# MGI-tech-bioinformatics/SuperPlus

Hardware: AMD Instinct MI355X
Metric: k-mers/s (DF createDict stage: trim + canonical k-mer count + solid filter + spectrum + adjacency) (higher is better)
Workload: dtype u64

## Files before the change

superplus_amd/csrc/dfk.hip:

```cpp
#include "../../include/dfk.h"
#include "dfk_kernels.h"

#include <algorithm>
#include <chrono>
#include <cstdarg>
#include <cstdio>
#include <cstdlib>
#include <cstring>
#include <atomic>
#include <fcntl.h>
#include <functional>
#include <new>
#include <string>
#include <sys/mman.h>
#include <sys/stat.h>
#include <unistd.h>
#include <condition_variable>
#include <memory>
#include <mutex>
#include <thread>
#include <vector>

using namespace dfk;

namespace {

thread_local std::string g_err;

int fail(int code, const char* fmt, ...)
{
    char buf[512];
    va_list ap; va_start(ap, fmt); vsnprintf(buf, sizeof buf, fmt, ap); va_end(ap);
    g_err = buf;
    return code;
}

#define HIP_TRY(expr) do { hipError_t e_ = (expr); if (e_ != hipSuccess) \
    return fail(DFK_E_HIP, "%s failed: %s (%s:%d)", #expr, hipGetErrorString(e_), __FILE__, __LINE__); } while (0)

template <class F> int guarded(F&& f)
{
    try { return f(); }
    catch (const std::bad_alloc&) { return fail(DFK_E_NOMEM, "out of host memory"); }
    catch (const std::exception& e) { return fail(DFK_E_HIP, "internal error: %s", e.what()); }
    catch (...) { return fail(DFK_E_HIP, "internal error"); }
}

struct DevBuf {
    void* p = nullptr; size_t bytes = 0;
    bool sub = false;
};

bool g_trace = getenv("DFK_TRACE") != nullptr;
#define TRACE(...) do { if (g_trace) { fprintf(stderr, "[dfk] " __VA_ARGS__); fputc('\n', stderr); fflush(stderr); } } while (0)
inline double wall_now() { return std::chrono::duration<double>(std::chrono::steady_clock::now().time_since_epoch()).count(); }

template <int K> struct CountCfg;
#ifndef DFK_LOG2S
#define DFK_LOG2S 11
#endif
#ifndef DFK_NWAVES
#define DFK_NWAVES 8
#endif
template <> struct CountCfg<40> { static constexpr int LOG2S = DFK_LOG2S, NWAVES = DFK_NWAVES; };
template <> struct CountCfg<48> { static constexpr int LOG2S = DFK_LOG2S, NWAVES = DFK_NWAVES; };
template <> struct CountCfg<60> { static constexpr int LOG2S = DFK_LOG2S, NWAVES = DFK_NWAVES; };

struct Inputs {
    const uint8_t* packed; uint64_t packed_bytes;
    const uint64_t* base_off; const uint32_t* read_len;
    const uint8_t* pq; uint64_t pq_bytes; const uint64_t* pq_off;
    const int32_t* bc; uint64_t n_reads;
};

}

struct dfk_ctx {
    dfk_config cfg{};
    int device = 0;
    hipStream_t stream = nullptr;
    hipStream_t stream2 = nullptr;
    hipDeviceProp_t prop{};
    uint64_t budget = 0, held = 0, peak = 0;
    struct Owned { void* p; uint64_t bytes, seq; };
    std::vector<Owned> owned;
    uint64_t alloc_seq = 0;
    bool have = false;
    uint64_t n_reads = 0;
    struct FileRange { const char* base; uint64_t bytes; int fd; uint64_t off; };
    std::vector<FileRange> file_ranges;
    DevBuf good_len;
    struct Part { DevBuf buf, pre; uint64_t n = 0; uint64_t blist = 0, n_blist = 0; bool listed = false; };
    bool want_blist = false;
    int pending_blist = -1;
    std::function<int()> after_count_launch;
    std::vector<Part> parts;
    uint64_t n_solid = 0, n_boundary = 0;
    unsigned seg_attempt = 0;
    double distinct_per_inst = 0.0;
    double plan_derate = 0.95;
    std::vector<int64_t> hist;
    std::vector<dfk_entry32> sorted, sorted_pre;
    bool sorted_ok = false, sorted_pre_ok = false;
    dfk_stats st{};
    bool shard_open = false, shard_use_bc = false;
    const void* sh_in[7] = {};
    uint64_t sh_packed_bytes = 0, sh_pq_bytes = 0, sh_n_reads = 0, sh_n_inst_local = 0;
    int64_t sh_read_id0 = 0;
    DevBuf shard_send[2];
    uint32_t shard_send_pass[2] = {~0u, ~0u};
    DevBuf shard_recv[2];
    unsigned shard_recv_seq = 0;
    uint64_t budget_taken = 0;
    void* sh_staged[6] = {};
    uint64_t sh_b0 = 0, sh_b1 = 0, sh_q0 = 0, sh_q1 = 0, sh_staged_reads = 0;
    DevBuf adj_keys, adj_src; uint64_t adj_n = 0;
    DevBuf set; uint64_t set_mask = 0;
    double t_upload_done = 0;
    uint32_t shard_world = 1, shard_log2_nb = 0;
    void* shard_state = nullptr;
    void (*shard_state_free)(void*) = nullptr;
    void* lane_pool = nullptr; void (*lane_pool_free)(void*) = nullptr;
    std::mutex lane_mu;
    void* graph_state = nullptr;
    void (*graph_state_free)(void*) = nullptr;
    unsigned int* d_resident = nullptr;
    unsigned int resident_target = 0;
    unsigned int last_wg_idle = 0;
    void* kept[6] = {};
    uint64_t kept_packed_bytes = 0, kept_pq_bytes = 0, kept_n_reads = 0, kept_budget = 0;

    struct Free { uint64_t off, bytes; };
    struct Chunk { char* p; uint64_t bytes; std::vector<Free> free_list; bool adopted = false; };
    std::vector<Chunk> chunks;
    uint64_t reserved = 0;

    uint64_t first_chunk_hint = 0;
    bool carve(Chunk& k, size_t bytes, DevBuf& b, bool long_lived)
    {
        if (!long_lived) {
            for (size_t i = k.free_list.size(); i-- > 0;)
                if (k.free_list[i].bytes >= bytes) {
                    k.free_list[i].bytes -= bytes;
                    b.p = k.p + k.free_list[i].off + k.free_list[i].bytes; b.bytes = bytes;
                    if (!k.free_list[i].bytes) k.free_list.erase(k.free_list.begin() + i);
                    return true;
                }
            return false;
        }
// ... 579 lines not shown
    }
    unsigned int bad = 0;
    HIP_TRY(hipMemcpy(&bad, J->d_bad.p, 4, hipMemcpyDeviceToHost));
    c->release(J->d_bad); c->release(J->cur);
    if (bad) return fail(DFK_E_HIP, "scatter: %u buckets did not receive the records counted for them (run summaries and bucket counters disagree)", bad);
    TRACE("scatter of buckets [%u, %u) done (%llu records, %llu items)", J->lo, J->lo + J->n,
          (unsigned long long)J->P.n_records, (unsigned long long)J->P.n_items);
    return 0;
}

constexpr int E_SPLIT_NO_ROOM = -101;
constexpr int E_SEGMENT_FULL = -100;

struct CountRun {
    CountGlobals* g = nullptr; uint4* seg = nullptr; unsigned long long* hist = nullptr;
    CountParams cp{}; unsigned grid = 0;
    DevBuf big; uint64_t big_cap = 0;
    DevBuf d_hist, d_g;
    DevBuf d_snap;
    DevBuf d_part;
    DevBuf d_wg;
    uint64_t solid_seen = 0, inst_seen = 0;
    uint64_t boundary_seen = 0;
    uint64_t splits_seen = 0;
};

int count_run_begin(dfk_ctx* c, CountRun* R)
{
    int rc = c->alloc(R->d_hist, (uint64_t)HIST_GLOBAL_BINS * 8, "spectrum bins", true); if (rc) return rc;
    rc = c->alloc(R->d_g, sizeof(CountGlobals), "count globals", true); if (rc) return rc;
    HIP_TRY(hipMemsetAsync(R->d_hist.p, 0, (uint64_t)HIST_GLOBAL_BINS * 8, c->stream));
    HIP_TRY(hipMemsetAsync(R->d_g.p, 0, sizeof(CountGlobals), c->stream));
    R->g = (CountGlobals*)R->d_g.p; R->hist = (unsigned long long*)R->d_hist.p;
    return c->alloc(R->d_snap, (uint64_t)HIST_GLOBAL_BINS * 8 + 256, "spectrum snapshot", true);
}

int count_snapshot(dfk_ctx* c, CountRun* R, bool restore)
{
    char* snap = (char*)R->d_snap.p;
    const uint64_t hb = (uint64_t)HIST_GLOBAL_BINS * 8;
    if (!restore) {
        HIP_TRY(hipMemcpyAsync(snap, R->d_hist.p, hb, hipMemcpyDeviceToDevice, c->stream));
        HIP_TRY(hipMemcpyAsync(snap + hb, R->d_g.p, sizeof(CountGlobals), hipMemcpyDeviceToDevice, c->stream));
    } else {
        HIP_TRY(hipMemcpyAsync(R->d_hist.p, snap, hb, hipMemcpyDeviceToDevice, c->stream));
        HIP_TRY(hipMemcpyAsync(R->d_g.p, snap + hb, sizeof(CountGlobals), hipMemcpyDeviceToDevice, c->stream));
    }
    return 0;
}

int count_run_end(dfk_ctx* c, CountRun* R)
{
    CountGlobals hg{};
    HIP_TRY(hipMemcpy(&hg, R->d_g.p, sizeof hg, hipMemcpyDeviceToHost));
    c->st.n_distinct = hg.n_distinct; c->n_boundary = hg.n_boundary;
#ifdef DFK_PHASE_TIMES
    {
        unsigned long long ph[16] = {};
        (void)hipMemcpyFromSymbol(ph, HIP_SYMBOL(g_phase), sizeof ph);
        unsigned long long tot = 0; for (int i = 0; i < 12; ++i) tot += ph[i];
        static const char* nm[12] = {"item loop tail (thread 0 publishes)", "barrier: item start", "chunks (stage + insert)", "barrier: chunks done", "finish pass 1 (solidity)", "barrier", "finish pass 2 (adjacency look-ups)", "barrier", "finish pass 3 (emit)", "barrier", "clear + reduce", "drain"};
        fprintf(stderr, "[dfk] k_count wave cycles by phase (%.3e memtime ticks in all):\n", (double)tot);
        for (int i = 0; i < 12; ++i) fprintf(stderr, "[dfk]   %5.1f %%  %s\n", 100.0 * (double)ph[i] / (double)std::max(1ull, tot), nm[i]);
        unsigned long long z[16] = {};
        (void)hipMemcpyToSymbol(HIP_SYMBOL(g_phase), z, sizeof z);
    }
#endif
    DevBuf d_max; int rc = c->alloc(d_max, 16, "max bin"); if (rc) return rc;
    HIP_TRY(hipMemsetAsync(d_max.p, 0, 16, c->stream));
    hipLaunchKernelGGL(k_hist_max, dim3(1024), dim3(256), 0, c->stream, (const unsigned long long*)R->d_hist.p, HIST_GLOBAL_BINS,
                       (unsigned int*)d_max.p);
    uint32_t nb = 0;
    HIP_TRY(hipMemcpyAsync(&nb, d_max.p, 4, hipMemcpyDeviceToHost, c->stream));
    HIP_TRY(hipStreamSynchronize(c->stream));
    c->hist.assign(nb, 0);
    if (nb) HIP_TRY(hipMemcpy(c->hist.data(), R->d_hist.p, 8ull * nb, hipMemcpyDeviceToHost));
    TRACE("spectrum read back: %u bins, %llu solid", nb, (unsigned long long)c->n_solid);
    c->release(d_max); c->release(R->d_hist); c->release(R->d_g); c->release(R->d_snap);
    return 0;
}

template <int K> unsigned count_grid(const dfk_ctx* c, int nbc = 1)
{
    constexpr int LOG2S = CountCfg<K>::LOG2S, NW = CountCfg<K>::NWAVES;
    const size_t lds = count_lds_bytes<K, LOG2S, NW, 1>() + (size_t)(nbc > 1 ? nbc - 1 : 0) * sizeof(uint32_t) * (1u << LOG2S);
    const unsigned per_cu = (unsigned)std::max<size_t>(1, (size_t)(160 * 1024) / lds);
    return (unsigned)c->prop.multiProcessorCount * per_cu;
}

int launch_boundary_list(dfk_ctx* c)
{
    if (c->pending_blist < 0) return 0;
    const dfk_ctx::Part& part = c->parts[(size_t)c->pending_blist];
    c->pending_blist = -1;
    unsigned long long* ctl = (unsigned long long*)((char*)part.buf.p + part.blist);
    HIP_TRY(hipMemsetAsync(ctl, 0, 16, c->stream2));
    hipLaunchKernelGGL(k_boundary_list, dim3((unsigned)std::min<uint64_t>((part.n + 2047) / 2048, 4096)), dim3(256), 0, c->stream2,
                       (const uint4*)part.buf.p, part.n, (uint32_t*)(ctl + 2), part.n_blist, ctl);
    HIP_TRY(hipGetLastError());
    return 0;
}

template <int K, int NBC>
int launch_count(dfk_ctx* c, const Partition& P, const ItemRange* d_items, uint64_t n_items, const CountRun& R,
                 std::vector<ItemRange>* overflowed, float* kernel_ms, const uint32_t* d_sub = nullptr, bool single_kmer_records = false)
{
    constexpr int LOG2S = CountCfg<K>::LOG2S, NW = CountCfg<K>::NWAVES;
    if (n_items == 0) return 0;
    if (n_items >= (1ull << 32)) return fail(DFK_E_ARG, "too many work items in one pass");
    DevBuf d_ovf;
    int rc = c->alloc(d_ovf, n_items * sizeof(ItemRange), "overflow list"); if (rc) return rc;
    HIP_TRY(hipMemsetAsync(&R.g->next_item, 0, 8, c->stream));
    HIP_TRY(hipMemsetAsync(&R.g->n_wg_idle, 0, 4, c->stream));
    CountParams cp = R.cp; cp.n_items = (uint32_t)n_items; cp.single = single_kmer_records ? 1u : 0u;
    const size_t lds = count_lds_bytes<K, LOG2S, NW, NBC>();
    auto kern = d_sub ? k_count<K, LOG2S, NW, NBC, true> : k_count<K, LOG2S, NW, NBC, false>;
    HIP_TRY(hipFuncSetAttribute(reinterpret_cast<const void*>(kern), hipFuncAttributeMaxDynamicSharedMemorySize, (int)lds));
    TRACE("k_count: %llu items, grid %u, lds %zu, seg_cap %llu", (unsigned long long)n_items, R.grid, lds, (unsigned long long)R.cp.seg_cap);
    Timer tk(c->stream);
    tk.start();
    hipLaunchKernelGGL(kern, dim3(R.grid), dim3(NW * 64), lds, c->stream,
                       (const uint4*)P.records.p, d_items, (const uint64_t*)P.base.p, cp, R.g, R.seg, (WgOut*)R.d_wg.p, R.hist,
                       (ItemRange*)d_ovf.p, d_sub, c->d_resident);
    HIP_TRY(hipGetLastError());
    c->resident_target += R.grid;
    if (c->after_count_launch || c->pending_blist >= 0) {
        hipLaunchKernelGGL(k_gate, dim3(1), dim3(64), 0, c->stream2, (const unsigned int*)c->d_resident, c->resident_target, 200000ull, c->d_resident + 1);
    }
    if (c->after_count_launch) { std::function<int()> f; f.swap(c->after_count_launch); rc = f(); if (rc) return rc; }
    rc = launch_boundary_list(c); if (rc) return rc;
    *kernel_ms += tk.stop();
    CountGlobals g{};
    HIP_TRY(hipMemcpyAsync(&g, R.g, sizeof g, hipMemcpyDeviceToHost, c->stream));
    HIP_TRY(hipStreamSynchronize(c->stream));
    c->last_wg_idle = g.n_wg_idle;
    if (g.n_overflow) {
        const size_t at = overflowed->size();
        overflowed->resize(at + g.n_overflow);
        HIP_TRY(hipMemcpy(overflowed->data() + at, d_ovf.p, sizeof(ItemRange) * g.n_overflow, hipMemcpyDeviceToHost));
    }
    c->release(d_ovf);
    return 0;
}

template <int K, int NBC>
int launch_count_big(dfk_ctx* c, const Partition& P, const std::vector<ItemRange>& singles, CountRun& R)
{
    constexpr int KW = KTraits<K>::KW, NW = 8;
    const uint32_t n = (uint32_t)singles.size();
    std::vector<uint32_t> idx(2 * n);
    for (uint32_t i = 0; i < n; ++i) { idx[2 * i] = singles[i].b0; idx[2 * i + 1] = singles[i].b1; }
    DevBuf d_idx, d_val;
    int rc = c->alloc(d_idx, 8ull * n, "gather index"); if (rc) return rc;
    rc = c->alloc(d_val, 16ull * n, "gather values"); if (rc) return rc;
    HIP_TRY(hipMemcpyAsync(d_idx.p, idx.data(), 8ull * n, hipMemcpyHostToDevice, c->stream));
    hipLaunchKernelGGL(k_gather_u64, dim3((2 * n + 255) / 256), dim3(256), 0, c->stream, (const uint64_t*)P.ipre.p,
                       (const uint32_t*)d_idx.p, 2 * n, (uint64_t*)d_val.p);
    HIP_TRY(hipGetLastError());
    std::vector<uint64_t> val(2 * n);
    HIP_TRY(hipMemcpyAsync(val.data(), d_val.p, 16ull * n, hipMemcpyDeviceToHost, c->stream));
    HIP_TRY(hipStreamSynchronize(c->stream));
    c->release(d_idx); c->release(d_val);
    std::vector<BigItem> items; uint64_t words = 0, tot_inst = 0;
    std::vector<uint64_t> chunk_pre(n + 1, 0), slot_pre(n + 1, 0), rec(2 * n);
    {
        DevBuf d_i2, d_v2;
        rc = c->alloc(d_i2, 8ull * n, "gather index"); if (rc) return rc;
        rc = c->alloc(d_v2, 16ull * n, "gather values"); if (rc) return rc;
        HIP_TRY(hipMemcpyAsync(d_i2.p, idx.data(), 8ull * n, hipMemcpyHostToDevice, c->stream));
        hipLaunchKernelGGL(k_gather_u64, dim3((2 * n + 255) / 256), dim3(256), 0, c->stream, (const uint64_t*)P.base.p,
                           (const uint32_t*)d_i2.p, 2 * n, (uint64_t*)d_v2.p);
        HIP_TRY(hipGetLastError());
        HIP_TRY(hipMemcpyAsync(rec.data(), d_v2.p, 16ull * n, hipMemcpyDeviceToHost, c->stream));
        HIP_TRY(hipStreamSynchronize(c->stream));
        c->release(d_i2); c->release(d_v2);
    }
    for (uint32_t i = 0; i < n; ++i) {
        tot_inst += val[2 * i + 1] - val[2 * i];
        chunk_pre[i + 1] = chunk_pre[i] + (rec[2 * i + 1] - rec[2 * i] + COUNT_CHUNK - 1) / COUNT_CHUNK;
    }
    double per_inst = c->distinct_per_inst > 0.0 ? std::min(1.0, std::max(0.05, 1.5 * c->distinct_per_inst)) : 1.0;
    DevBuf d_items, d_fail, d_pre;
    {
        const uint64_t more = tot_inst / std::max<uint32_t>(1, c->cfg.min_freq) + 1;
        if (!R.big.p) { R.big_cap = more; rc = c->alloc(R.big, R.big_cap * 32, "fallback solid entries"); if (rc) return rc; }
        else {
            CountGlobals g0{};
            HIP_TRY(hipMemcpy(&g0, R.d_g.p, sizeof g0, hipMemcpyDeviceToHost));
            DevBuf grown;
            rc = c->alloc(grown, (g0.big_cursor + more) * 32, "fallback solid entries"); if (rc) return rc;
// ... 1374 lines not shown
```

superplus_amd/csrc/dfk_kernels.h:

```cpp
#pragma once
#include <type_traits>
#include "dfk_device.h"

namespace dfk {

template <int K>
__global__ void __launch_bounds__(256)
k_trim(const uint8_t* __restrict__ pq, const uint64_t* __restrict__ pq_off, uint64_t pq_nbytes,
       const uint64_t* __restrict__ base_off, uint64_t packed_bytes, const uint32_t* __restrict__ read_len,
       uint64_t n_reads, uint32_t min_qual, uint32_t* __restrict__ good_len,
       unsigned long long* __restrict__ n_inst, unsigned int* __restrict__ bad,
       unsigned long long* __restrict__ sum_good)
{
    unsigned long long mine = 0, good = 0;
    bool any_bad = false;
    for (uint64_t r = (uint64_t)blockIdx.x * blockDim.x + threadIdx.x; r < n_reads; r += (uint64_t)gridDim.x * blockDim.x) {
        uint32_t gl = 0;
        uint64_t p = pq_off[r], end = pq_off[r + 1];
        uint32_t idx = 0, run = 0;
        const uint64_t b0 = base_off[r], b1 = base_off[r + 1];
        bool ok = p <= end && end <= pq_nbytes && b0 <= b1 && b1 <= packed_bytes && b1 - b0 >= ((uint64_t)read_len[r] + 3) / 4;
        if (!ok) end = p;
        while (p < end) {
            uint32_t nQs = pq[p];
// ... 14 lines not shown
                    const uint64_t by = bit >> 3;
                    const uint32_t sh = (uint32_t)(bit & 7);
                    uint64_t w = 0;
                    if (by + 8 <= pq_nbytes) __builtin_memcpy(&w, pq + by, 8);
                    else for (uint32_t k = 0; k < 8 && by + k < pq_nbytes; ++k) w |= (uint64_t)pq[by + k] << (8 * k);
                    w >>= sh;
                    const uint32_t n = min(left, (64u - sh) / nBits);
                    for (uint32_t i = 0; i < n; ++i, w >>= nBits) {
                        const uint32_t q = minQ + ((uint32_t)w & fmask);
                        if (q < min_qual) run = 0;
                        else if (++run >= (uint32_t)K) gl = idx + 1;
                        ++idx;
                    }
                    bit += (uint64_t)n * nBits; left -= n;
                }
            }
            p += blk;
        }
        uint32_t rl = read_len[r];
        if (!ok || idx != rl) { any_bad = true; gl = 0; }
        if (gl > rl) gl = rl;
        good_len[r] = gl;
        good += gl;
        if (gl >= (uint32_t)K + 1) mine += gl - K + 1;
    }
    __shared__ unsigned long long sh[2][4];
    __shared__ unsigned int sh_bad;
    if (threadIdx.x == 0) sh_bad = 0;
    __syncthreads();
#pragma unroll
    for (int d = 32; d > 0; d >>= 1) { mine += __shfl_down(mine, d, 64); good += __shfl_down(good, d, 64); }
    if ((threadIdx.x & 63) == 0) { sh[0][threadIdx.x >> 6] = mine; sh[1][threadIdx.x >> 6] = good; }
    if (any_bad) atomicOr(&sh_bad, 1u);
    __syncthreads();
    if (threadIdx.x == 0) {
        unsigned long long a0 = sh[0][0] + sh[0][1] + sh[0][2] + sh[0][3], a1 = sh[1][0] + sh[1][1] + sh[1][2] + sh[1][3];
        if (a0) atomicAdd(n_inst, a0);
        if (a1) atomicAdd(sum_good, a1);
        if (sh_bad) atomicOr(bad, 1u);
    }
}

struct PartParams {
    uint32_t M;
    uint32_t W;
    uint32_t log2_nb;
    uint32_t log2_world;
    int64_t  read_id0;
    uint32_t sub_lo;
    uint32_t sub_n;
    uint32_t class_mask;
};

constexpr uint32_t SWEEP_CLASSES = 32;
__host__ __device__ inline uint32_t sweep_class_of(uint32_t local_bucket, uint32_t log2_local)
{ return log2_local > 5 ? local_bucket >> (log2_local - 5) : local_bucket; }
__host__ __device__ inline uint32_t sweep_class_mask(uint32_t sub_lo, uint32_t sub_n, uint32_t log2_local)
{
    if (sub_n == 0) return 0u;
    const uint32_t a = sweep_class_of(sub_lo, log2_local), b = sweep_class_of(sub_lo + sub_n - 1, log2_local);
    const uint32_t upto_b = b >= 31 ? 0xFFFFFFFFu : ((1u << (b + 1)) - 1u);
    return upto_b & ~((1u << a) - 1u);
}

constexpr int PART_THREADS = 128;
constexpr int PART_RING = 2;
constexpr int SUMMARY_RUNS = 10;
constexpr uint32_t SUMMARY_OVERFLOW = 15;

__device__ __forceinline__ uint32_t pass_local(uint32_t bucket, const PartParams& pp)
{
    const uint32_t ls = pp.log2_nb - pp.log2_world;
    const uint32_t d = (bucket & ((1u << ls) - 1u)) - pp.sub_lo;
    return d < pp.sub_n ? (bucket >> ls) * pp.sub_n + d : 0xFFFFFFFFu;
}

__device__ __forceinline__ uint32_t bucket_of(uint32_t minhash, const PartParams& pp)
{
    const uint32_t b = (minhash * 0x9E3779B1u) >> (32 - pp.log2_nb);
    return ((b & ((1u << pp.log2_world) - 1u)) << (pp.log2_nb - pp.log2_world)) | (b >> pp.log2_world);
}
constexpr int PART_QCAP = 8;

template <int K>
__device__ __forceinline__ void emit_record(const uint32_t* __restrict__ words, uint64_t n_words, uint64_t bit0,
                                            uint32_t s0, uint32_t nk, uint32_t bucket, uint32_t gl, int32_t tag,
                                            uint64_t dst_index, uint4* __restrict__ records)
{
    const bool hp = s0 > 0;
    const bool hs = s0 + nk + (uint32_t)K <= gl;
    uint64_t bo = bit0 + 2ull * (hp ? s0 - 1 : 0);
    uint64_t wi = bo >> 5; uint32_t sh = (uint32_t)bo & 31u;
    uint32_t w[7];
#pragma unroll
    for (int i = 0; i < 7; ++i) w[i] = (wi + i < n_words) ? words[wi + i] : 0u;
    uint32_t o[6];
#pragma unroll
    for (int i = 0; i < 6; ++i) o[i] = alignbit(w[i + 1], w[i], sh);
    if (!hp) {
#pragma unroll
        for (int i = 5; i > 0; --i) o[i] = (o[i] << 2) | (o[i - 1] >> 30);
        o[0] <<= 2;
    }
    uint32_t nbits = 2u * (1u + nk + (uint32_t)K - 1u + (hs ? 1u : 0u));
#pragma unroll
    for (int i = 0; i < 6; ++i) {
        uint32_t lo = 32u * i;
        if (nbits <= lo) o[i] = 0;
        else if (nbits < lo + 32u) o[i] &= (1u << (nbits - lo)) - 1u;
    }
    uint4 a{rec_header(nk, hp, hs, bucket), (uint32_t)tag, o[0], o[1]};
    uint4 b{o[2], o[3], o[4], o[5]};
    records[2 * dst_index] = a;
    records[2 * dst_index + 1] = b;
}

constexpr uint32_t PART_CLASSES = 64;
__device__ __forceinline__ uint32_t class_bin(uint32_t bucket, const PartParams& pp)
{
    const uint32_t ls = pp.log2_nb - pp.log2_world;
    const uint32_t sub = bucket & ((1u << ls) - 1u);
    return (bucket >> ls) * PART_CLASSES + (ls > 6 ? sub >> (ls - 6) : sub);
}

template <int K, bool WRITE>
__device__ __forceinline__ void
partition_read(uint64_t r, uint32_t* smem, uint32_t* __restrict__ lh,
            const uint8_t* __restrict__ packed, uint64_t packed_bytes, const uint64_t* __restrict__ base_off,
            const uint32_t* __restrict__ good_len, const int32_t* __restrict__ bc, int64_t ign_bc_below,
            uint64_t n_reads, const PartParams& pp,
            unsigned long long* __restrict__ bucket_acc, unsigned long long* __restrict__ bucket_cur, uint64_t n_out,
            uint4* __restrict__ records, uint4* __restrict__ summaries, const uint32_t* __restrict__ read_list, uint64_t n_list,
            const uint64_t* __restrict__ slice_base, uint32_t* __restrict__ read_classes)
{
    auto place = [&](uint32_t b) -> uint64_t {
        if (!slice_base) { const uint64_t d = atomicAdd(&bucket_cur[b], 1ull); return d < n_out ? d : ~0ull; }
        const uint32_t owner = b / pp.sub_n;
        const uint64_t d = slice_base[owner] + atomicAdd(&bucket_cur[owner], 1ull);
        return d < slice_base[owner + 1] ? d : ~0ull;
    };
    uint32_t* arr = smem;
    uint32_t* queue = smem + pp.W * PART_THREADS;
    uint8_t* sidx = reinterpret_cast<uint8_t*>(smem + pp.W * PART_THREADS);
    uint32_t* ring = reinterpret_cast<uint32_t*>(sidx + pp.W * PART_THREADS);
    uint64_t sum_lo = 0, sum_hi = 0;
    const int tid = threadIdx.x;
    if (WRITE && read_list) { if (r >= n_list) return; r = read_list[r]; }
    const uint32_t M = pp.M, W = pp.W;
    const uint32_t gl = r < n_reads ? good_len[r] : 0;
    if (gl < (uint32_t)K + 1) {
        if (!WRITE && r < n_reads) { summaries[r] = uint4{0, 0, 0, 0}; if (read_classes) read_classes[r] = 0u; }
        return;
    }
    uint32_t Pi = 0, cur_rel = 0;
    uint32_t cmask = 0;
    const uint32_t log2_local = pp.log2_nb - pp.log2_world;

    const uint64_t byte0 = base_off[r];
    const uint32_t* words = reinterpret_cast<const uint32_t*>(packed);
    const uint64_t n_words = (packed_bytes + 3) >> 2;
    const uint64_t bit0 = byte0 * 8;
    int32_t tag = -1;
    if (bc && (int64_t)r + pp.read_id0 >= ign_bc_below) tag = bc[r];

    const uint32_t mmask = M == 16 ? 0xFFFFFFFFu : ((1u << (2 * M)) - 1u);
    const uint32_t rsh = 2 * (M - 1);
    uint32_t f = 0, rc = 0;
    uint32_t P = 0;
    uint32_t bi = 0;
    uint32_t cur_b = 0, cur_s0 = 0, cur_nk = 0;
    uint32_t qn = 0;

    uint64_t wi = bit0 >> 5;
    uint64_t filled_to = wi;
    auto fill = [&]() {
        uint32_t w[PART_RING];
#pragma unroll
        for (int k = 0; k < PART_RING; ++k) w[k] = filled_to + k < n_words ? words[filled_to + k] : 0u;
#pragma unroll
        for (int k = 0; k < PART_RING; ++k) ring[((filled_to + k) & (PART_RING - 1)) * PART_THREADS + tid] = w[k];
        filled_to += PART_RING;
    };
    uint32_t wbits, wnext = 0;
    if (!WRITE) { fill(); wbits = ring[(wi & (PART_RING - 1)) * PART_THREADS + tid]; }
    else { wbits = wi < n_words ? words[wi] : 0u; wnext = wi + 1 < n_words ? words[wi + 1] : 0u; }
    uint32_t wpos = (uint32_t)bit0 & 31u;
    uint32_t sfx_next = 0xFFFFFFFFu;

    auto close_run = [&]() {
        if (WRITE && cur_b == 0xFFFFFFFFu) return;
        if (!WRITE) {
            if (lh) { const uint32_t bin = class_bin(cur_b, pp); atomicAdd(&lh[bin], 1u); atomicAdd(&lh[(PART_CLASSES << pp.log2_world) + bin], cur_nk); }
            else atomicAdd(&bucket_acc[cur_b], (1ull << 32) | cur_nk);
            cmask |= 1u << sweep_class_of(cur_b & ((1u << log2_local) - 1u), log2_local);
            if (qn < (uint32_t)SUMMARY_RUNS) {
                const uint64_t fld = cur_nk | (cur_rel << 6);
                const uint32_t b = 8u + 12u * qn;
// ... 474 lines not shown
    uint32_t s0 = 0;
#pragma unroll
    for (int i = 0; i < SUMMARY_RUNS; ++i) {
        if ((uint32_t)i < n) {
            constexpr int B0 = 8;
            const int b = B0 + 12 * i;
            const uint32_t fld = (uint32_t)(b + 12 <= 64 ? lo >> b : b >= 64 ? hi >> (b - 64) : (lo >> b) | (hi << (64 - b))) & 0xFFFu;
            const uint32_t nk = fld & 63u, rel = fld >> 6;
            const uint64_t bo = bit0 + 2ull * (s0 + rel);
            const uint64_t wi = bo >> 5;
            const uint32_t w0 = words[wi], w1 = wi + 1 < n_words ? words[wi + 1] : 0u;
            const uint32_t x = alignbit(w1, w0, (uint32_t)bo & 31u) & mmask;
            uint32_t y = __brev(x);
            y = ((y >> 1) & 0x55555555u) | ((y & 0x55555555u) << 1);
            const uint32_t fw = y >> (32 - 2 * M), rcv = ~x & mmask;
            const uint32_t bucket = bucket_of(mmer_hash(fw < rcv ? fw : rcv), pp);
            const uint32_t lb = pass_local(bucket, pp);
            if (lb != 0xFFFFFFFFu) f(s0, nk, lb, bucket >> (pp.log2_nb - pp.log2_world), bit0, (uint32_t)i + 1 == n);
            s0 += nk;
        }
    }
}

template <int K>
__global__ void __launch_bounds__(256)
k_scatter_slices(const uint8_t* __restrict__ packed, uint64_t packed_bytes, const uint64_t* __restrict__ base_off,
                 const uint32_t* __restrict__ good_len, const int32_t* __restrict__ bc, int64_t ign_bc_below,
                 uint64_t n_reads, PartParams pp, const uint4* __restrict__ summaries, const uint32_t* __restrict__ read_classes,
                 const uint64_t* __restrict__ slice_base,
                 unsigned long long* __restrict__ slice_fill,
                 uint4* __restrict__ records)
{
    __shared__ uint32_t cnt[256];
    __shared__ unsigned long long at[256];
    __shared__ uint16_t list[256 * SLICE_READS];
    __shared__ uint32_t n_list;
    const uint32_t world = 1u << pp.log2_world;
    const int lane = threadIdx.x & 63;
    const uint64_t r_block = (uint64_t)blockIdx.x * 256 * SLICE_READS;
    if (threadIdx.x < world) cnt[threadIdx.x] = 0;
    if (threadIdx.x == 0) n_list = 0;
    __syncthreads();
#pragma unroll
    for (int j = 0; j < SLICE_READS; ++j) {
        const uint32_t rel = 256u * j + threadIdx.x;
        const uint64_t r = r_block + rel;
        const bool hit = r < n_reads && (!read_classes || (read_classes[r] & pp.class_mask) != 0u);
        const unsigned long long mk = __ballot(hit);
        uint32_t w = 0;
        if (lane == 0 && mk) w = atomicAdd(&n_list, (uint32_t)__popcll(mk));
        w = __builtin_amdgcn_readfirstlane(w);
        if (hit) list[w + __popcll(mk & ((1ull << lane) - 1ull))] = (uint16_t)rel;
    }
    __syncthreads();
    const uint32_t n = n_list;
    for (uint32_t i = threadIdx.x; i < n; i += 256)
        for_each_run_in_pass<K, false>(r_block + list[i], packed, packed_bytes, base_off, pp, summaries,
                                       [&](uint32_t, uint32_t, uint32_t, uint32_t owner, uint64_t, bool) { atomicAdd(&cnt[owner], 1u); });
    __syncthreads();
    if (threadIdx.x < world) {
        const uint32_t m = cnt[threadIdx.x];
        at[threadIdx.x] = slice_base[threadIdx.x] + (m ? atomicAdd(&slice_fill[threadIdx.x], (unsigned long long)m) : 0ull);
        cnt[threadIdx.x] = 0;
    }
    __syncthreads();
    const uint32_t* words = reinterpret_cast<const uint32_t*>(packed);
    const uint64_t n_words = (packed_bytes + 3) >> 2;
    (void)good_len;
    for (uint32_t i = threadIdx.x; i < n; i += 256) {
        const uint64_t r = r_block + list[i];
        int32_t tag = -1;
        if (bc && (int64_t)r + pp.read_id0 >= ign_bc_below) tag = bc[r];
        for_each_run_in_pass<K, true>(r, packed, packed_bytes, base_off, pp, summaries,
            [&](uint32_t s0, uint32_t nk, uint32_t lb, uint32_t owner, uint64_t bit0, bool last) {
                const uint64_t dst = at[owner] + atomicAdd(&cnt[owner], 1u);
                if (dst < slice_base[owner + 1]) emit_record<K>(words, n_words, bit0, s0, nk, lb, last ? 0u : 0xFFFFFFFFu, tag, dst, records);
            });
    }
}

#ifndef DFK_SWEEP_READS
#define DFK_SWEEP_READS 8
#endif
template <int K> constexpr int sweep_reads() { return KTraits<K>::KW == 4 ? 2 : DFK_SWEEP_READS; }
template <int K>
__global__ void __launch_bounds__(256)
k_scatter_runs(const uint8_t* __restrict__ packed, uint64_t packed_bytes, const uint64_t* __restrict__ base_off,
               const uint32_t* __restrict__ good_len, const int32_t* __restrict__ bc, int64_t ign_bc_below,
               uint64_t n_reads, PartParams pp, const uint4* __restrict__ summaries, const uint32_t* __restrict__ read_classes,
               unsigned long long* __restrict__ bucket_cur, uint64_t n_out, uint4* __restrict__ records)
{
    constexpr int SWEEP_READS = sweep_reads<K>();
    __shared__ uint16_t list[256 * SWEEP_READS];
    __shared__ uint32_t n_list;
    (void)good_len;
    const int lane = threadIdx.x & 63;
    const uint64_t r_block = (uint64_t)blockIdx.x * 256 * SWEEP_READS;
    if (threadIdx.x == 0) n_list = 0;
    __syncthreads();
#pragma unroll
    for (int j = 0; j < SWEEP_READS; ++j) {
        const uint32_t rel = 256u * j + threadIdx.x;
        const uint64_t r = r_block + rel;
        const bool hit = r < n_reads && (read_classes[r] & pp.class_mask) != 0u;
        const unsigned long long mk = __ballot(hit);
        uint32_t at = 0;
        if (lane == 0 && mk) at = atomicAdd(&n_list, (uint32_t)__popcll(mk));
        at = __builtin_amdgcn_readfirstlane(at);
        if (hit) list[at + __popcll(mk & ((1ull << lane) - 1ull))] = (uint16_t)rel;
    }
    __syncthreads();
    const uint32_t n = n_list;
    const uint32_t* words = reinterpret_cast<const uint32_t*>(packed);
    const uint64_t n_words = (packed_bytes + 3) >> 2;
    for (uint32_t i = threadIdx.x; i < n; i += 256) {
        const uint64_t r = r_block + list[i];
        int32_t tag = -1;
        if (bc && (int64_t)r + pp.read_id0 >= ign_bc_below) tag = bc[r];
        for_each_run_in_pass<K, true>(r, packed, packed_bytes, base_off, pp, summaries,
            [&](uint32_t s0, uint32_t nk, uint32_t lb, uint32_t, uint64_t bit0, bool last) {
                const uint64_t dst = atomicAdd(&bucket_cur[lb], 1ull);
                if (dst < n_out) emit_record<K>(words, n_words, bit0, s0, nk, lb, last ? 0u : 0xFFFFFFFFu, tag, dst, records);
            });
    }
}



struct ItemRange { uint32_t b0, b1; };

struct CountParams {
    uint32_t min_freq, min_bc;
    uint32_t n_items;
    uint32_t single;
    uint64_t seg_cap;
    uint32_t do_adj;
    uint32_t keep_pre;
};

struct CountGlobals {
    unsigned long long n_distinct;
    unsigned long long big_cursor;
    unsigned int next_item;
    unsigned int n_overflow;
    unsigned int solid_overflow;
    unsigned int n_split;
    unsigned long long n_boundary;
    unsigned long long part_cursor;
    unsigned int n_wg_idle;
    unsigned int pad_idle;
};

struct WgOut { unsigned long long chunk; unsigned int used; unsigned int pad; };

constexpr int COUNT_HIST_BINS = 256;
constexpr uint32_t COUNT_MAX_PROBE = 96;
constexpr uint32_t HIST_GLOBAL_BINS = 1u << 24;
constexpr int COUNT_CHUNK = 32;
constexpr uint32_t FLAG_SOLID = 0x80000000u;

template <int K> struct WaveStage {
    uint32_t rec[COUNT_CHUNK * 8 + 8];
    uint32_t starts[COUNT_CHUNK];
    uint32_t msk[64];
    uint32_t pc[64];
};

__device__ __forceinline__ uint32_t tld(const uint32_t* p)
{ return __hip_atomic_load(p, __ATOMIC_RELAXED, __HIP_MEMORY_SCOPE_AGENT); }
__device__ __forceinline__ void tst(uint32_t* p, uint32_t v)
{ __hip_atomic_store(p, v, __ATOMIC_RELAXED, __HIP_MEMORY_SCOPE_AGENT); }

struct Probe {
    uint32_t k0, k1, k2, k3, ctx, fp, step, slot;
    int32_t tag;
    bool active;
};

__device__ __forceinline__ Probe probe_begin(u128 c, uint32_t ctx, int32_t tag, uint32_t S, bool active)
{
    const uint32_t h = key_hash(c);
    return Probe{(uint32_t)c.lo, (uint32_t)(c.lo >> 32), (uint32_t)c.hi, (uint32_t)(c.hi >> 32), ctx, (h >> 24) | 1u,
                 ((h >> 11) | 1u) & (S - 1), h & (S - 1), tag, active};
}

#define DFK_COMPILER_FENCE() asm volatile("" ::: "memory")
#ifdef DFK_PHASE_TIMES
__device__ unsigned long long g_phase[16];
struct PhaseClock {
    unsigned long long t, acc[12];
    __device__ __forceinline__ void start() { t = __builtin_amdgcn_s_memtime(); for (int i = 0; i < 12; ++i) acc[i] = 0; }
    __device__ __forceinline__ void mark(int i) { const unsigned long long n = __builtin_amdgcn_s_memtime(); acc[i] += n - t; t = n; }
    __device__ __forceinline__ void flush(int lane) { if (lane == 0) for (int i = 0; i < 12; ++i) atomicAdd(&g_phase[i], acc[i]); }
};
#define PH(i) phase.mark(i)
#else
#define PH(i) do { } while (0)
#endif
__device__ unsigned int g_big_fail[4];

enum : uint32_t { PS_PROBING = 0, PS_FOUND = 1, PS_FAILED = 2, PS_IDLE = 3 };
constexpr uint32_t PROBE_COST = 1u << 12, PROBE_LIMIT = (COUNT_MAX_PROBE + 1) * PROBE_COST;

template <int KW, int NBC, bool LDS_TABLE>
__device__ __forceinline__ bool table_insert(uint32_t* __restrict__ keys, uint32_t* __restrict__ cnt,
                                             uint32_t* __restrict__ ctxs, uint32_t* __restrict__ bcw,
// ... 1402 lines not shown
```

Before: 64.65 billion.

## Rework scatter sweep with per-wave compaction and raise count kernel waves

Replaces the block-level LDS read list in k_scatter_runs with per-wave ballot/ds_permute compaction, so each lane handles one in-pass read. Each read is processed by a new sweep_read that prefetches the minimizer words for all runs before hashing them, then loads and stores record words as vector quads. It also raises the default count-kernel waves to 10 when two workgroups still fit in a CU's LDS, and adds launch bounds for occupancy. This is meant to cut LDS synchronisation and serialized per-run loads in the scatter, at the cost of more registers and extra unaligned vector loads.

```diff
diff --git a/superplus_amd/csrc/dfk.hip b/superplus_amd/csrc/dfk.hip
--- a/superplus_amd/csrc/dfk.hip
+++ b/superplus_amd/csrc/dfk.hip
@@ -59,12 +59,22 @@
 #ifndef DFK_LOG2S
 #define DFK_LOG2S 11
 #endif
+template <> struct CountCfg<40> { static constexpr int LOG2S = DFK_LOG2S; };
+template <> struct CountCfg<48> { static constexpr int LOG2S = DFK_LOG2S; };
+template <> struct CountCfg<60> { static constexpr int LOG2S = DFK_LOG2S; };
 #ifndef DFK_NWAVES
-#define DFK_NWAVES 8
+#define DFK_NWAVES 10
 #endif
-template <> struct CountCfg<40> { static constexpr int LOG2S = DFK_LOG2S, NWAVES = DFK_NWAVES; };
-template <> struct CountCfg<48> { static constexpr int LOG2S = DFK_LOG2S, NWAVES = DFK_NWAVES; };
-template <> struct CountCfg<60> { static constexpr int LOG2S = DFK_LOG2S, NWAVES = DFK_NWAVES; };
+constexpr size_t CU_LDS_BYTES = 160 * 1024;
+template <int K> constexpr size_t count_lds_bytes_nbc(int nwaves, int nbc)
+{
+    return count_lds_bytes<K, CountCfg<K>::LOG2S, 0, 1>() + (size_t)(nbc > 1 ? nbc - 1 : 0) * sizeof(uint32_t) * (1u << CountCfg<K>::LOG2S)
+           + sizeof(WaveStage<K>) * (size_t)nwaves;
+}
+template <int K> constexpr int count_waves(int nbc) { return 2 * count_lds_bytes_nbc<K>(DFK_NWAVES, nbc) <= CU_LDS_BYTES ? DFK_NWAVES : 8; }
+static_assert(DFK_NWAVES >= 8 && 2 * DFK_NWAVES <= 24, "two k_count workgroups leave the sweep at least 8 of a CU's 32 wave slots");
+static_assert(count_lds_bytes_nbc<48>(count_waves<48>(3), 3) == count_lds_bytes<48, DFK_LOG2S, count_waves<48>(3), 3>(), "count_lds_bytes_nbc");
+static_assert(count_waves<60>(1) == 8, "K=60: two 8-wave workgroups are all a CU's LDS holds");
 
 struct Inputs {
     const uint8_t* packed; uint64_t packed_bytes;
@@ -810,9 +820,8 @@
 
 template <int K> unsigned count_grid(const dfk_ctx* c, int nbc = 1)
 {
-    constexpr int LOG2S = CountCfg<K>::LOG2S, NW = CountCfg<K>::NWAVES;
-    const size_t lds = count_lds_bytes<K, LOG2S, NW, 1>() + (size_t)(nbc > 1 ? nbc - 1 : 0) * sizeof(uint32_t) * (1u << LOG2S);
-    const unsigned per_cu = (unsigned)std::max<size_t>(1, (size_t)(160 * 1024) / lds);
+    const size_t lds = count_lds_bytes_nbc<K>(count_waves<K>(nbc), nbc);
+    const unsigned per_cu = (unsigned)std::max<size_t>(1, CU_LDS_BYTES / lds);
     return (unsigned)c->prop.multiProcessorCount * per_cu;
 }
 
@@ -833,7 +842,7 @@
 int launch_count(dfk_ctx* c, const Partition& P, const ItemRange* d_items, uint64_t n_items, const CountRun& R,
                  std::vector<ItemRange>* overflowed, float* kernel_ms, const uint32_t* d_sub = nullptr, bool single_kmer_records = false)
 {
-    constexpr int LOG2S = CountCfg<K>::LOG2S, NW = CountCfg<K>::NWAVES;
+    constexpr int LOG2S = CountCfg<K>::LOG2S, NW = count_waves<K>(NBC);
     if (n_items == 0) return 0;
     if (n_items >= (1ull << 32)) return fail(DFK_E_ARG, "too many work items in one pass");
     DevBuf d_ovf;
diff --git a/superplus_amd/csrc/dfk_kernels.h b/superplus_amd/csrc/dfk_kernels.h
--- a/superplus_amd/csrc/dfk_kernels.h
+++ b/superplus_amd/csrc/dfk_kernels.h
@@ -120,37 +120,63 @@
 }
 constexpr int PART_QCAP = 8;
 
+struct __attribute__((packed, aligned(4))) WordPair { uint32_t x, y; };
+struct __attribute__((packed, aligned(4))) WordQuad { uint32_t x, y, z, w; };
+__device__ __forceinline__ uint2 load_pair(const uint32_t* p) { const WordPair v = *reinterpret_cast<const WordPair*>(p); return uint2{v.x, v.y}; }
+__device__ __forceinline__ uint4 load_quad(const uint32_t* p) { const WordQuad v = *reinterpret_cast<const WordQuad*>(p); return uint4{v.x, v.y, v.z, v.w}; }
+
+__device__ __forceinline__ void record_load(const uint32_t* __restrict__ words, uint64_t n_words, uint64_t bit0, uint32_t s0, uint32_t (&w)[7])
+{
+    const uint64_t wi = (bit0 + 2ull * (s0 > 0 ? s0 - 1 : 0)) >> 5;
+    if (wi + 7 <= n_words) {
+        const uint4 a = load_quad(words + wi);
+        const uint4 b = load_quad(words + wi + 3);
+        w[0] = a.x; w[1] = a.y; w[2] = a.z; w[3] = b.x; w[4] = b.y; w[5] = b.z; w[6] = b.w;
+    } else {
+#pragma unroll
+        for (int i = 0; i < 7; ++i) w[i] = (wi + i < n_words) ? words[wi + i] : 0u;
+    }
+}
+
+template <int K>
+__device__ __forceinline__ void record_store(const uint32_t (&w)[7], uint64_t bit0,
+                                             uint32_t s0, uint32_t nk, uint32_t bucket, uint32_t gl, int32_t tag,
+                                             uint64_t dst_index, uint64_t n_out, uint4* __restrict__ records)
+{
+    const bool hp = s0 > 0;
+    const bool hs = s0 + nk + (uint32_t)K <= gl;
+    const uint32_t sh = (uint32_t)(bit0 + 2ull * (hp ? s0 - 1 : 0)) & 31u;
+    uint32_t o[6];
+#pragma unroll
+    for (int i = 0; i < 6; ++i) o[i] = alignbit(w[i + 1], w[i], sh);
+    if (!hp) {
+#pragma unroll
+        for (int i = 5; i > 0; --i) o[i] = (o[i] << 2) | (o[i - 1] >> 30);
+        o[0] <<= 2;
+    }
+    uint32_t nbits = 2u * (1u + nk + (uint32_t)K - 1u + (hs ? 1u : 0u));
+#pragma unroll
+    for (int i = 0; i < 6; ++i) {
+        uint32_t lo = 32u * i;
+        if (nbits <= lo) o[i] = 0;
+        else if (nbits < lo + 32u) o[i] &= (1u << (nbits - lo)) - 1u;
+    }
+    uint4 a{rec_header(nk, hp, hs, bucket), (uint32_t)tag, o[0], o[1]};
+    uint4 b{o[2], o[3], o[4], o[5]};
+    if (dst_index < n_out) {
+        records[2 * dst_index] = a;
+        records[2 * dst_index + 1] = b;
+    }
+}
+
 template <int K>
 __device__ __forceinline__ void emit_record(const uint32_t* __restrict__ words, uint64_t n_words, uint64_t bit0,
                                             uint32_t s0, uint32_t nk, uint32_t bucket, uint32_t gl, int32_t tag,
                                             uint64_t dst_index, uint4* __restrict__ records)
 {
-    const bool hp = s0 > 0;
-    const bool hs = s0 + nk + (uint32_t)K <= gl;
-    uint64_t bo = bit0 + 2ull * (hp ? s0 - 1 : 0);
-    uint64_t wi = bo >> 5; uint32_t sh = (uint32_t)bo & 31u;
     uint32_t w[7];
-#pragma unroll
-    for (int i = 0; i < 7; ++i) w[i] = (wi + i < n_words) ? words[wi + i] : 0u;
-    uint32_t o[6];
-#pragma unroll
-    for (int i = 0; i < 6; ++i) o[i] = alignbit(w[i + 1], w[i], sh);
-    if (!hp) {
-#pragma unroll
-        for (int i = 5; i > 0; --i) o[i] = (o[i] << 2) | (o[i - 1] >> 30);
-        o[0] <<= 2;
-    }
-    uint32_t nbits = 2u * (1u + nk + (uint32_t)K - 1u + (hs ? 1u : 0u));
-#pragma unroll
-    for (int i = 0; i < 6; ++i) {
-        uint32_t lo = 32u * i;
-        if (nbits <= lo) o[i] = 0;
-        else if (nbits < lo + 32u) o[i] &= (1u << (nbits - lo)) - 1u;
-    }
-    uint4 a{rec_header(nk, hp, hs, bucket), (uint32_t)tag, o[0], o[1]};
-    uint4 b{o[2], o[3], o[4], o[5]};
-    records[2 * dst_index] = a;
-    records[2 * dst_index + 1] = b;
+    record_load(words, n_words, bit0, s0, w);
+    record_store<K>(w, bit0, s0, nk, bucket, gl, tag, dst_index, ~0ull, records);
 }
 
 constexpr uint32_t PART_CLASSES = 64;
@@ -791,46 +817,118 @@
 #ifndef DFK_SWEEP_READS
 #define DFK_SWEEP_READS 8
 #endif
-template <int K> constexpr int sweep_reads() { return KTraits<K>::KW == 4 ? 2 : DFK_SWEEP_READS; }
+template <int K> constexpr int sweep_reads() { return DFK_SWEEP_READS; }
+
+__device__ __forceinline__ uint32_t summary_field(uint64_t lo, uint64_t hi, int i)
+{
+    const int b = 8 + 12 * i;
+    return (uint32_t)(b + 12 <= 64 ? lo >> b : b >= 64 ? hi >> (b - 64) : (lo >> b) | (hi << (64 - b))) & 0xFFFu;
+}
+
 template <int K>
-__global__ void __launch_bounds__(256)
+__device__ __forceinline__ void sweep_read(uint64_t r, const uint32_t* __restrict__ words, uint64_t n_words,
+                                           const uint64_t* __restrict__ base_off, const int32_t* __restrict__ bc, int64_t ign_bc_below,
+                                           const PartParams& pp, const uint4* __restrict__ summaries,
+                                           unsigned long long* __restrict__ bucket_cur, uint64_t n_out, uint4* __restrict__ records)
+{
+    const uint4 sm = summaries[r];
+    const uint64_t bit0 = base_off[r] * 8;
+    int32_t tag = -1;
+    if (bc) { const int32_t v = bc[r]; if ((int64_t)r + pp.read_id0 >= ign_bc_below) tag = v; }
+    const uint32_t n = (sm.x & 15u) == SUMMARY_OVERFLOW ? 0u : sm.x & 15u;
+    uint64_t lo = (uint64_t)sm.x | ((uint64_t)sm.y << 32), hi = (uint64_t)sm.z | ((uint64_t)sm.w << 32);
+    const uint32_t M = pp.M;
+    const uint32_t mmask = M == 16 ? 0xFFFFFFFFu : ((1u << (2 * M)) - 1u);
+    uint2 mw[SUMMARY_RUNS];
+    const uint64_t last_pair = n_words >= 2 ? n_words - 2 : 0;
+    {
+        uint32_t s0 = 0;
+#pragma unroll
+        for (int i = 0; i < SUMMARY_RUNS; ++i) {
+            const uint32_t fld = summary_field(lo, hi, i);
+            const uint64_t wi = (bit0 + 2ull * (s0 + (fld >> 6))) >> 5;
+            mw[i] = uint2{0u, 0u};
+            if ((uint32_t)i < n) mw[i] = load_pair(words + (wi + 2 <= n_words ? wi : last_pair));
+            s0 += fld & 63u;
+        }
+    }
+    uint32_t lbs[SUMMARY_RUNS], in_pass = 0;
+    {
+        uint32_t s0 = 0;
+#pragma unroll
+        for (int i = 0; i < SUMMARY_RUNS; ++i) {
+            const uint32_t fld = summary_field(lo, hi, i);
+            const uint64_t bo = bit0 + 2ull * (s0 + (fld >> 6));
+            const bool at_end = (bo >> 5) + 2 > n_words;
+            const uint32_t x = alignbit(at_end ? 0u : mw[i].y, at_end ? mw[i].y : mw[i].x, (uint32_t)bo & 31u) & mmask;
+            uint32_t y = __brev(x);
+            y = ((y >> 1) & 0x55555555u) | ((y & 0x55555555u) << 1);
+            const uint32_t fw = y >> (32 - 2 * M), rcv = ~x & mmask;
+            lbs[i] = pass_local(bucket_of(mmer_hash(fw < rcv ? fw : rcv), pp), pp);
+            if ((uint32_t)i < n && lbs[i] != 0xFFFFFFFFu) in_pass |= 1u << i;
+            s0 += fld & 63u;
+            __builtin_amdgcn_sched_barrier(0);
+        }
+    }
+    while (in_pass) {
+        asm volatile("" : "+v"(lo), "+v"(hi));
+        const uint32_t idx = (uint32_t)__builtin_ctz(in_pass);
+        in_pass &= in_pass - 1u;
+        uint32_t s0 = 0, nk = 0, lb = 0;
+#pragma unroll
+        for (int i = 0; i < SUMMARY_RUNS; ++i) {
+            const uint32_t nki = summary_field(lo, hi, i) & 63u;
+            if ((uint32_t)i < idx) s0 += nki;
+            if ((uint32_t)i == idx) { nk = nki; lb = lbs[i]; }
+        }
+        const uint64_t dst = atomicAdd(&bucket_cur[lb], 1ull);
+        uint32_t w[7];
+        record_load(words, n_words, bit0, s0, w);
+        record_store<K>(w, bit0, s0, nk, lb, idx + 1u == n ? 0u : 0xFFFFFFFFu, tag, dst, n_out, records);
+    }
+}
+
+template <int K>
+__global__ void __launch_bounds__(256, 8)
 k_scatter_runs(const uint8_t* __restrict__ packed, uint64_t packed_bytes, const uint64_t* __restrict__ base_off,
                const uint32_t* __restrict__ good_len, const int32_t* __restrict__ bc, int64_t ign_bc_below,
                uint64_t n_reads, PartParams pp, const uint4* __restrict__ summaries, const uint32_t* __restrict__ read_classes,
                unsigned long long* __restrict__ bucket_cur, uint64_t n_out, uint4* __restrict__ records)
 {
     constexpr int SWEEP_READS = sweep_reads<K>();
-    __shared__ uint16_t list[256 * SWEEP_READS];
-    __shared__ uint32_t n_list;
+    static_assert(SWEEP_READS >= 1 && SWEEP_READS < 32, "a lane keeps one bit per read of its");
     (void)good_len;
-    const int lane = threadIdx.x & 63;
-    const uint64_t r_block = (uint64_t)blockIdx.x * 256 * SWEEP_READS;
-    if (threadIdx.x == 0) n_list = 0;
-    __syncthreads();
-#pragma unroll
-    for (int j = 0; j < SWEEP_READS; ++j) {
-        const uint32_t rel = 256u * j + threadIdx.x;
-        const uint64_t r = r_block + rel;
-        const bool hit = r < n_reads && (read_classes[r] & pp.class_mask) != 0u;
-        const unsigned long long mk = __ballot(hit);
-        uint32_t at = 0;
-        if (lane == 0 && mk) at = atomicAdd(&n_list, (uint32_t)__popcll(mk));
-        at = __builtin_amdgcn_readfirstlane(at);
-        if (hit) list[at + __popcll(mk & ((1ull << lane) - 1ull))] = (uint16_t)rel;
-    }
-    __syncthreads();
-    const uint32_t n = n_list;
+    const uint32_t lane = threadIdx.x & 63u;
+    const uint64_t r_wave = ((uint64_t)blockIdx.x * 4u + (uint32_t)__builtin_amdgcn_readfirstlane((int)(threadIdx.x >> 6))) * (64u * SWEEP_READS);
     const uint32_t* words = reinterpret_cast<const uint32_t*>(packed);
     const uint64_t n_words = (packed_bytes + 3) >> 2;
-    for (uint32_t i = threadIdx.x; i < n; i += 256) {
-        const uint64_t r = r_block + list[i];
-        int32_t tag = -1;
-        if (bc && (int64_t)r + pp.read_id0 >= ign_bc_below) tag = bc[r];
-        for_each_run_in_pass<K, true>(r, packed, packed_bytes, base_off, pp, summaries,
-            [&](uint32_t s0, uint32_t nk, uint32_t lb, uint32_t, uint64_t bit0, bool last) {
-                const uint64_t dst = atomicAdd(&bucket_cur[lb], 1ull);
-                if (dst < n_out) emit_record<K>(words, n_words, bit0, s0, nk, lb, last ? 0u : 0xFFFFFFFFu, tag, dst, records);
-            });
+    uint32_t cm[SWEEP_READS];
+    if (r_wave + 64u * SWEEP_READS <= n_reads) {
+#pragma unroll
+        for (int j = 0; j < SWEEP_READS; ++j) cm[j] = read_classes[r_wave + 64u * j + lane];
+    } else {
+#pragma unroll
+        for (int j = 0; j < SWEEP_READS; ++j) { const uint64_t r = r_wave + 64u * j + lane; cm[j] = r < n_reads ? read_classes[r] : 0u; }
+    }
+    uint32_t hits = 0;
+#pragma unroll
+    for (int j = 0; j < SWEEP_READS; ++j) if ((cm[j] & pp.class_mask) != 0u) hits |= 1u << j;
+    uint32_t q = 0, qn = 0;
+#pragma unroll 1
+    for (int j = 0; j <= SWEEP_READS; ++j) {
+        const bool hit = (hits >> j) & 1u;
+        const unsigned long long mk = __ballot(hit);
+        const uint32_t c = (uint32_t)__popcll(mk);
+        const unsigned long long mine = hit ? mk : ~mk;
+        const uint32_t p = (hit ? 0u : c) + __builtin_amdgcn_mbcnt_hi((uint32_t)(mine >> 32), __builtin_amdgcn_mbcnt_lo((uint32_t)mine, 0u));
+        const uint32_t t = (uint32_t)__builtin_amdgcn_ds_permute((int)(((qn + p) & 63u) << 2), (int)(64u * j + lane));
+        const uint32_t tot = qn + c;
+        if (lane >= qn && lane < tot) q = t;
+        if (tot >= 64u || (j == SWEEP_READS && tot != 0u)) {
+            if (lane < tot) sweep_read<K>(r_wave + q, words, n_words, base_off, bc, ign_bc_below, pp, summaries, bucket_cur, n_out, records);
+            q = t;
+            qn = tot >= 64u ? tot - 64u : 0u;
+        } else qn = tot;
     }
 }
 
```

Measured after the change: 50.54 billion. 0.782x the previous value.
